# dmlc/difacto

Measured on AMD Instinct MI355X. Metric: examples/sec (FM SGD worker step, Criteo-shape, V_dim=64), higher is better.
Workload: dtype f32

## Files before the change

### difacto_amd/capi.py

```python
import ctypes as C
import os

import numpy as np

_HERE = os.path.dirname(os.path.abspath(__file__))
LIB_PATH = os.environ.get("DIFACTO_HIP_LIB") or os.path.join(_HERE, "libdifacto_hip.so")

FEA_COUNT, WEIGHT, GRADIENT = 1, 2, 3
INIT_REFRAND, INIT_HASH = 0, 1
U64MAX = 2 ** 64 - 1

SYMBOLS = [
    "dfh_last_error", "dfh_updater_param_default", "dfh_ctx_create", "dfh_ctx_destroy", "dfh_ctx_sync",
    "dfh_ctx_stream", "dfh_ctx_device", "dfh_reverse_bytes", "dfh_encode_fea_grp_id", "dfh_table_create",
    "dfh_table_destroy", "dfh_table_size", "dfh_table_param", "dfh_table_bytes", "dfh_pull", "dfh_push",
    "dfh_table_export", "dfh_table_import", "dfh_fm_predict", "dfh_fm_calcgrad", "dfh_loss_evaluate",
    "dfh_auc_times_n", "dfh_batch_create", "dfh_batch_destroy", "dfh_batch_load_host", "dfh_batch_load_device",
    "dfh_localize", "dfh_batch_load_localized_host", "dfh_batch_get_localized", "dfh_batch_shape", "dfh_sgd_step",
    "dfh_batch_progress", "dfh_batch_get_pred", "dfh_row_stride", "dfh_shard_pull", "dfh_shard_push_count",
    "dfh_shard_push_grad", "dfh_batch_forward", "dfh_batch_backward", "dfh_batch_device_keys", "dfh_malloc",
    "dfh_free", "dfh_memcpy_h2d", "dfh_memcpy_d2h", "dfh_ctx_set_timing", "dfh_ctx_get_timing", "dfh_kernel_name",
    "dfh_table_warm_start", "dfh_ctx_set_pipeline", "dfh_batch_lookup", "dfh_localize_lookup", "dfh_rowbuf_create", "dfh_rowbuf_destroy", "dfh_rowbuf_load_host", "dfh_batch_gather_rows", "dfh_batch_set_option", "dfh_batch_key_ranges", "dfh_batch_attach_device",
    "dfh_batch_key_ranges_device", "dfh_shard_resolve", "dfh_shard_pull_resolved", "dfh_shard_push_count_resolved",
    "dfh_shard_push_grad_resolved", "dfh_table_check", "dfh_ctx_set_timing_mask", "dfh_table_save", "dfh_table_load", "dfh_shard_resolve_multi", "dfh_shard_push_count_multi",
    "dfh_shard_push_grad_multi", "dfh_shard_count_pull_multi", "dfh_shard_push_grad_listed", "dfh_shard_release", "dfh_ctx_set_option", "dfh_table_set_has_aux", "dfh_table_has_aux",
    "dfh_comm_unique_id", "dfh_comm_create_rccl", "dfh_comm_create_callback", "dfh_comm_destroy", "dfh_comm_rank", "dfh_comm_world",
    "dfh_comm_allreduce_sum", "dfh_shard_create", "dfh_shard_destroy", "dfh_shard_owned_range", "dfh_shard_step", "dfh_shard_prefetch_counts",
    "dfh_shard_pull_host", "dfh_shard_push_host", "dfh_comm_allgather", "dfh_shard_balanced_splits", "dfh_shard_set_exchange", "dfh_shard_set_timing", "dfh_shard_get_timing",
    "dfh_comm_stats", "dfh_comm_info", "dfh_comm_selfcheck", "dfh_comm_wire_probe", "dfh_table_capacity", "dfh_batch_prepare_rows", "dfh_rowbuf_load_host_slices",
    "dfh_rowbuf_set_labels", "dfh_batch_prepare_cached", "dfh_batch_get_rows",
    "dfh_batch_create_many", "dfh_shard_multi_words", "dfh_shard_reserve", "dfh_comm_create_loopback", "dfh_comm_loopback_feed", "dfh_comm_loopback_wire", "dfh_comm_loopback_wire_time",
    "dfh_vec_inner_multi", "dfh_vec_combine", "dfh_vec_line_step", "dfh_lbfgs_create", "dfh_lbfgs_destroy", "dfh_lbfgs_add_chunk",
    "dfh_lbfgs_init_model", "dfh_lbfgs_shape", "dfh_lbfgs_get_model", "dfh_lbfgs_set_weights", "dfh_lbfgs_calc_grad",
# ... 625 lines not shown
    def load_localized_host(self, offset, index, value, label, feaids, feacnt=None):
        offset = np.ascontiguousarray(offset, np.uint64)
        index = np.ascontiguousarray(index, np.uint32)
        value = None if value is None else np.ascontiguousarray(value, np.float32)
        label = np.ascontiguousarray(label, np.float32)
        feaids = np.ascontiguousarray(feaids, np.uint64)
        feacnt = None if feacnt is None else np.ascontiguousarray(feacnt, np.float32)
        _ck(lib().dfh_batch_load_localized_host(self.h, len(offset) - 1, _p(offset), _p(index), _p(value), _p(label),
                                                _p(feaids), _p(feacnt), len(feaids)))

    def shape(self, want_U=True):
        a, b, c = C.c_size_t(0), C.c_size_t(0), C.c_size_t(0)
        _ck(lib().dfh_batch_shape(self.h, C.byref(a), C.byref(b), C.byref(c) if want_U else None))
        return a.value, b.value, c.value

    def get_localized(self):
        nrows, nnz, U = self.shape()
        feaids = np.zeros(max(U, 1), np.uint64)
        cnt = np.zeros(max(U, 1), np.float32)
        index = np.zeros(max(nnz, 1), np.uint32)
        u = C.c_size_t(0)
        _ck(lib().dfh_batch_get_localized(self.h, C.byref(u), _p(feaids), _p(cnt), _p(index)))
        return dict(U=U, feaids=feaids[:U], feacnt=cnt[:U], index=index[:nnz])

    def get_rows(self):
        nrows, _, _ = self.shape(want_U=False)
        off = np.zeros(nrows + 1, np.uint32)
        lab = np.zeros(nrows, np.float32)
        _ck(lib().dfh_batch_get_rows(self.h, _p(off), _p(lab)))
        return off, lab
# ... 428 lines not shown
```

### difacto_amd/csrc/dfh_api.hip

```cpp
#include <algorithm>
#include <chrono>
#include <cstring>
#include <mutex>
#include <new>
#include <thread>

#include <hip/hip_ext.h>
#include <rocprim/rocprim.hpp>

#include "dfh_kernels.hip"
#include "dfh_localize.hip"
#include "dfh_update.hip"
#include "dfh_riders.hip"

using namespace dfh;

namespace dfh {
static thread_local std::string g_err;
void set_error(const std::string& msg) { g_err = msg; }
}

struct dfh_ctx {
  int device = 0;
  hipStream_t stream = nullptr;
// ... 10 lines not shown
  int num_cu = 256;
  int fwd_depth = 5;
  int fwd_blocks = 0;
  int bwd_small_blocks = 2048;
  int upd_kernel = 1;
  int upd_hot_blocks = 512, upd_mid_blocks = 512, upd_few_blocks = 1024, upd_single_blocks = 4096;
  int upd_interleave = 0;
  int owner_per_key = 0;
  int upd_split = 1;
  int auc_in_update = 1;
  int shard_mixed_update = 1;
  int grow_initial_rows = 1 << 20;
  int event_flags = 1;
  int prep_priority = -1;
  int single_queue = 0;
  int rider_slot[4] = {2, 0, 1, 2};
  int rider_alone[4] = {0, 0, 0, 0};
  int rider_period[3] = {1, 1, 1};
  int rider_start[3] = {0, 0, 0};
  std::vector<dfh_batch*> pend;
  std::thread warm;

  uint32_t timing = 0;
  struct Span { int id; hipEvent_t a, b; int ride = 0; };
  std::vector<Span> spans;
  std::vector<hipEvent_t> pool;
  double t_ms[DFH_K_COUNT] = {0};
  uint64_t t_calls[DFH_K_COUNT] = {0};
};

// ... 111 lines not shown
  uint32_t auc_pending_n = 0;
  bool force_radix = false;
  bool force_sort_fallback = false;
  dfh_table* looked_up = nullptr;
  struct GatherSeg { struct dfh_rowbuf* rb; size_t at, n; };
  std::vector<GatherSeg> gsegs;
  GatherSrc gsrc{};
  bool gather_pending = false, gather_fusable = false, gather_any_value = false, loc_fuse_gather = false;
  const uint32_t *g_rows = nullptr, *g_off = nullptr;
  const float* g_lab = nullptr;
  LocView loc_v{};
  EmitOut loc_o{};
  uint32_t loc_gsort = 0;
  bool loc_big = false;
  int pend_stage = RID_STAGES;
};

namespace dfh {
namespace chunks {
inline hipError_t reset_prog(dfh_batch* b, hipStream_t s);
}
}

namespace {
int flush_pending(dfh_batch* b);
void pend_remove(dfh_ctx* c, dfh_batch* b);
inline hipStream_t prep_of(const dfh_batch* b) {
  const dfh_ctx* c = b->ctx;
  return (c->pipeline && b->prep) ? b->prep : c->stream;
}
// ... 820 lines not shown
  } else if (n == "shard_mixed_update") {
    DFH_ARG(value == 0 || value == 1, "shard_mixed_update must be 0 or 1");
    c->shard_mixed_update = value;
  } else if (n == "owner_per_key") {
    DFH_ARG(value == 0 || value == 1, "owner_per_key must be 0 (count push, Pull, gradient push per received entry) or 1 (per distinct key)");
    c->owner_per_key = value;
  } else if (n == "upd_split") {
    DFH_ARG(value == 0 || value == 1, "upd_split must be 0 (one block per hot key, whatever its length) or 1 (a block per part of 1 024 occurrences)");
    c->upd_split = value;
  } else if (n == "upd_interleave") {
    DFH_ARG(value >= 0 && value <= 64, "upd_interleave must be in [0, 64]");
    c->upd_interleave = value;
  } else if (n == "event_flags") {
    DFH_ARG(value == 0 || value == 1, "event_flags must be 0 (default events) or 1 (no system-scope fence); set before batches are created");
    c->event_flags = value;
  } else if (n == "single_queue") {
    DFH_ARG(value == 0 || value == 1, "single_queue must be 0 (preparation streams) or 1 (the Localizer's stages ride in the step's launches)");
    if (value != c->single_queue) {
      for (dfh_batch* p : std::vector<dfh_batch*>(c->pend)) {
        int rcf = flush_pending(p);
        if (rcf) return rcf;
      }
      int rcs = sync_all(c);
      if (rcs) return rcs;
      if (value) {
        c->nprep = 0;
        c->next_prep = 0;
        c->pipeline = false;
      }
      c->single_queue = value;
// ... 1138 lines not shown
}

int dfh_batch_destroy(dfh_batch* b) {
  if (b && b->n_prof)
    fprintf(stderr, "dfh_batch_prepare_rows x %llu: begin %.4f s, wait staged %.4f, write description %.4f, gather %.4f, localize %.4f, lookup + ready %.4f\n",
            (unsigned long long)b->n_prof, b->t_prof[0], b->t_prof[1], b->t_prof[2], b->t_prof[3], b->t_prof[4], b->t_prof[5]);
  if (!b) return DFH_OK;
  hipSetDevice(b->ctx->device);
  pend_remove(b->ctx, b);
  sync_all(b->ctx);
  if (b->ev_ready) hipEventDestroy(b->ev_ready);
  if (b->ev_free) hipEventDestroy(b->ev_free);
  if (b->ev_staged) hipEventDestroy(b->ev_staged);
  if (b->h_stage) hipHostFree(b->h_stage);
  if (b->d_xv) hipFree(b->d_xv);
  if (b->arena) hipFree(b->arena);
  if (b->shared_arena) {
    SharedArena* sa = static_cast<SharedArena*>(b->shared_arena);
    if (--sa->refs == 0) {
      hipFree(sa->base);
      delete sa;
    }
  }
  delete b;
  return DFH_OK;
}

}

#include "dfh_textparse.hip"
// ... 74 lines not shown
      else if (b->loc_fuse_gather) hipLaunchKernelGGL(k_loc_count_gather<LOC_MAX_BUCKETS>, dim3(v.ntiles), dim3(LOC_TILE_THREADS), 0, s, v, b->gsrc);
      else hipLaunchKernelGGL(k_loc_count<LOC_MAX_BUCKETS>, dim3(v.ntiles), dim3(LOC_TILE_THREADS), 0, s, v);
      break;
    case RID_SCATTER:
      if (b->loc_big) hipLaunchKernelGGL(k_loc_scatter<LOC_BIG_BUCKETS>, dim3(v.ntiles), dim3(LOC_TILE_THREADS), 0, s, v);
      else hipLaunchKernelGGL(k_loc_scatter<LOC_MAX_BUCKETS>, dim3(v.ntiles), dim3(LOC_TILE_THREADS), 0, s, v);
      break;
    case RID_SORT:
      hipLaunchKernelGGL(k_loc_sort, dim3(b->loc_gsort), dim3(LOC_SORT_THREADS), loc_sort_smem(), s, v);
      break;
    default:
      if (probe) hipLaunchKernelGGL(k_loc_emit<true>, dim3(b->loc_gsort), dim3(LOC_EMIT_THREADS), 0, s, v, b->loc_o, probe->v, b->d_urow);
      else hipLaunchKernelGGL(k_loc_emit<false>, dim3(b->loc_gsort), dim3(LOC_EMIT_THREADS), 0, s, v, b->loc_o, TableView{}, (uint32_t*)nullptr);
      break;
  }
}

void pend_remove(dfh_ctx* c, dfh_batch* b) {
  auto it = std::find(c->pend.begin(), c->pend.end(), b);
  if (it != c->pend.end()) c->pend.erase(it);
}

int flush_pending(dfh_batch* b) {
  dfh_ctx* c = b->ctx;
  if (b->pend_stage >= RID_STAGES) return DFH_OK;
  {
    TimeScope ts(c, DFH_K_LOCALIZE);
    for (int st = b->pend_stage; st < RID_STAGES; ++st) launch_loc_stage(b, st, c->stream);
  }
  b->pend_stage = RID_STAGES;
// ... 55 lines not shown
}

int localize_impl(dfh_batch* b, uint64_t max_index, dfh_table* probe) {
  dfh_ctx* c = b->ctx;
  DFH_HIP(hipSetDevice(c->device));
  const uint32_t N = (uint32_t)b->nnz;
  if (probe && N) {
    if (int rcr = table_reserve(probe, N)) return rcr;
  }
  {
    int rc = prep_begin(b);
    if (rc) return rc;
  }
  hipStream_t s = prep_of(b);
  b->looked_up = nullptr;
  if (b->pend_stage < RID_STAGES) {
    int rc = flush_pending(b);
    if (rc) return rc;
  }
  if (N == 0) {
    if (b->gather_pending) {
      int rcg = gather_alone(b, s);
      if (rcg) return rcg;
    }
    DFH_HIP(hipMemsetAsync(b->d_U, 0, 64 * sizeof(uint32_t), s));
    DFH_HIP(hipMemsetAsync(b->d_col_ptr, 0, 4, s));
    b->seg_nb = 0;
    b->localized = true;
    return prep_end(b);
  }
// ... 67 lines not shown
    o.sl.few = b->d_few;
    o.sl.few_ent = b->d_few_ent;
    v.split_n = b->d_U + 2;
    b->loc_big = big;
#ifndef DFH_LOC_GRID_CAP
#define DFH_LOC_GRID_CAP 1024
#endif
    b->loc_gsort = (unsigned)std::min<int>(P, big ? LOC_BIG_BUCKETS : DFH_LOC_GRID_CAP);
    if (cold && P > 1) {
      const uint32_t S = (uint32_t)P * LOC_OVERSAMPLE;
      const uint32_t nt = (S + 255) / 256;
      hipLaunchKernelGGL(k_ss_sample, dim3(nt), dim3(256), 0, s, v);
      hipLaunchKernelGGL(k_ss_rank, dim3(nt * nt), dim3(256), 0, s, v);
      hipLaunchKernelGGL(k_loc_splitters, dim3(nt), dim3(256), 0, s, v);
    }
    if (c->single_queue && !cold && !big && !probe) {
      b->pend_stage = 0;
      c->pend.push_back(b);
    } else {
      for (int st = 0; st < RID_STAGES; ++st) {
        launch_loc_stage(b, st, s, probe);
        if (st == RID_COUNT && b->loc_fuse_gather) {
          int rcg = gather_queued(b, s);
          b->loc_fuse_gather = false;
          if (rcg) return rcg;
        }
      }
    }
    b->spl_P = P;
    b->seg_nb = (uint32_t)P;
  } else {
// ... 153 lines not shown

int dfh_batch_shape(dfh_batch* b, size_t* nrows, size_t* nnz, size_t* U) {
  DFH_ARG(b, "NULL batch");
  if (nrows) *nrows = b->nrows;
  if (nnz) *nnz = b->nnz;
  if (U) {
    DFH_ARG(b->localized, "batch is not localized");
    uint32_t u = 0;
    int rc = flush_pending(b);
    if (rc) return rc;
    rc = sync_all(b->ctx);
    if (rc) return rc;
    DFH_HIP(hipMemcpyAsync(&u, b->d_U, 4, hipMemcpyDeviceToHost, b->ctx->stream));
    DFH_HIP(hipStreamSynchronize(b->ctx->stream));
    *U = u;
  }
  return DFH_OK;
}

int dfh_batch_get_localized(dfh_batch* b, size_t* U, uint64_t* feaids, float* feacnt, uint32_t* index) {
  DFH_ARG(b && b->localized, "batch is not localized");
  size_t u = 0;
  int rc = dfh_batch_shape(b, nullptr, nullptr, &u);
  if (rc) return rc;
  if (U) *U = u;
  hipStream_t s = b->ctx->stream;
  if (feaids && u) DFH_HIP(hipMemcpyAsync(feaids, b->d_feaids, u * 8, hipMemcpyDeviceToHost, s));
  if (feacnt && u) {
    if (!b->has_cnt) {
      hipLaunchKernelGGL(k_loc_counts, dim3(grid_for_threads(u, b->ctx)), dim3(256), 0, s, b->d_col_ptr, b->d_U, b->d_feacnt);
// ... 241 lines not shown
```

### difacto_amd/csrc/dfh_localize.hip

```cpp
#ifndef DFH_LOCALIZE_HIP_
#define DFH_LOCALIZE_HIP_
#include "dfh_internal.h"
#include "dfh_feed_layout.h"

namespace dfh {

constexpr int LOC_OVERSAMPLE = 8;
constexpr int LOC_MAX_BUCKETS = 1024;
constexpr int LOC_BIG_BUCKETS = 4096;
constexpr int LOC_AVG_BUCKET = 384;
constexpr int LOC_MIN_AVG = 48;
constexpr int LOC_MAX_AVG = 700;
constexpr int LOC_LDS_CAP = 1024;
#ifndef DFH_LOC_TILE_THREADS
#define DFH_LOC_TILE_THREADS 1024
#endif
constexpr int LOC_TILE_THREADS = DFH_LOC_TILE_THREADS;
constexpr int LOC_PER_THREAD = LOC_TILE / LOC_TILE_THREADS;
constexpr int LOC_SORT_THREADS = 256;
constexpr int LOC_EMIT_THREADS = 256;

struct LocView {
  const uint64_t* raw;
  uint32_t n;
// ... 23 lines not shown
  uint64_t* last_key;
  uint32_t* nheads;
  uint32_t* lh;
  uint32_t* split_n;
};

struct SegListsOut {
  uint2* mid;
  SegEnt* mid_ent;
  uint2* hot;
  SegEnt* hot_ent;
  uint2* few;
  SegEnt* few_ent;
};

__device__ __forceinline__ uint64_t make_key(uint64_t id, uint64_t max_index) {
  const uint64_t m = (max_index == ~0ULL) ? (id == ~0ULL ? 0ULL : id) : id % max_index;
  return reverse_bytes(m);
}

constexpr int LOC_XCDS = 8;

__device__ __forceinline__ bool comp_less(uint64_t ka, uint32_t pa, uint64_t kb, uint32_t pb) {
  return ka < kb || (ka == kb && pa < pb);
}

template <bool MAX>
__device__ __forceinline__ uint32_t wave_inclusive(uint32_t x) {
#define DFH_DPP_STEP(ctrl, row_mask)                                                                      \
  {                                                                                                       \
// ... 219 lines not shown
    v.run_off[bid * P + b] = h ? atomicAdd(&v.btotal[(bid & (LOC_XCDS - 1)) * MAXB + b], h) : 0u;
  }
}

template <int MAXB>
__global__ void __launch_bounds__(LOC_TILE_THREADS) k_loc_count(LocView v) {
  __shared__ __attribute__((aligned(16))) char smem[loc_count_smem<MAXB>()];
  loc_count_block<MAXB, LOC_TILE_THREADS>(v, blockIdx.x, gridDim.x, smem);
}
template <int MAXB>
__global__ void __launch_bounds__(LOC_TILE_THREADS) k_loc_count_gather(LocView v, GatherSrc g) {
  __shared__ __attribute__((aligned(16))) char smem[loc_count_smem<MAXB>() + loc_gather_smem()];
  loc_count_block<MAXB, LOC_TILE_THREADS, true>(v, blockIdx.x, gridDim.x, smem, &g);
}

__global__ void __launch_bounds__(LOC_DESC_ROWS) k_loc_describe(const uint32_t* __restrict__ src_off, const float* __restrict__ src_lab,
                                                                const uint32_t* __restrict__ h_rows, const uint32_t* __restrict__ h_base,
                                                                uint32_t n, uint32_t* __restrict__ dst_off, float* __restrict__ dst_lab,
                                                                int write_end) {
  __shared__ uint32_t wsum[LOC_DESC_ROWS / 64];
  const uint32_t q = blockIdx.x * LOC_DESC_ROWS + threadIdx.x;
  const bool in = q < n;
  const uint32_t r = h_rows[in ? q : n - 1u];
  const uint32_t lo = src_off[r], hi = src_off[r + 1u];
  const float lab = src_lab[r];
  const uint32_t len = in ? hi - lo : 0u;
  const uint32_t at = h_base[blockIdx.x] + block_exclusive_scan<LOC_DESC_ROWS / 64>(len, wsum, nullptr);
  if (in) {
    dst_off[q] = at;
    dst_lab[q] = lab;
// ... 118 lines not shown
    khi = take ? ohi : khi;
    tag = take ? ot : tag;
  }
}
template <int K, int J>
__device__ __forceinline__ void loc_net_merge(uint32_t& klo, uint32_t& khi, uint32_t& tag) {
  loc_net_stage<K, J>(klo, khi, tag);
  if constexpr (J > 1) loc_net_merge<K, J / 2>(klo, khi, tag);
}
template <int K = 2>
__device__ __forceinline__ void loc_net_sort64(uint32_t& klo, uint32_t& khi, uint32_t& tag) {
  loc_net_merge<K, K / 2>(klo, khi, tag);
  if constexpr (K < 64) loc_net_sort64<K * 2>(klo, khi, tag);
}

__device__ __forceinline__ bool loc_sort_bucket_lds(const LocView& v, uint32_t beg, uint32_t n, uint64_t* ak, uint32_t* ap,
                                                    uint64_t* bk, uint32_t* bp) {
  const uint64_t* gk = v.bkeys + beg;
  const uint32_t* gp = v.bpos + beg;
  uint64_t* sk = bk;
  uint32_t* sp = bp;
  const uint32_t lane = threadIdx.x & 63;
  for (uint32_t c0 = (threadIdx.x >> 6) * 64; c0 < n; c0 += LOC_SORT_THREADS) {
    const uint32_t idx = c0 + lane;
    const bool valid = idx < n;
    const uint64_t mk = valid ? gk[idx] : ~0ULL;
    uint32_t klo = (uint32_t)mk, khi = (uint32_t)(mk >> 32);
    uint32_t mp = valid ? gp[idx] : ~0u;
    loc_net_sort64(klo, khi, mp);
    if (valid) {
      bk[idx] = ((uint64_t)khi << 32) | klo;
      bp[idx] = mp;
    }
  }
  __syncthreads();
  constexpr int E = LOC_LDS_CAP / LOC_SORT_THREADS;
  constexpr int G = 2;
  static_assert(E * LOC_SORT_THREADS == LOC_LDS_CAP && E % G == 0 && LOC_SORT_THREADS % 64 == 0,
                "a thread carries E elements of a full bucket, G at a time");
  uint64_t* dk = ak;
  uint32_t* dp = ap;
  uint32_t sh = 6;
  for (uint32_t L = 64; L < n; L <<= 1, ++sh) {
// ... 27 lines not shown
      for (int e = 0; e < G; ++e) {
        const uint32_t idx = threadIdx.x + (g + e) * LOC_SORT_THREADS;
        if (idx < n) {
          const uint32_t dst = idx + at[e] - min((idx & ~(L - 1u)) | L, n);
          dk[dst] = mk[e];
          dp[dst] = mp[e];
        }
      }
    }
    __syncthreads();
    uint64_t* tk = sk; sk = dk; dk = tk;
    uint32_t* tp = sp; sp = dp; dp = tp;
  }
  return sk == ak;
}
__device__ __forceinline__ void loc_sort_bucket_global(const LocView& v, uint32_t beg, uint32_t n) {
  uint64_t* xk = v.bkeys + beg;
  uint32_t* xp = v.bpos + beg;
  uint64_t* yk = v.skeys + beg;
  uint32_t* yp = v.spos + beg;
  const uint32_t lane = threadIdx.x & 63;
  for (uint32_t c0 = (threadIdx.x >> 6) * 64; c0 < n; c0 += LOC_SORT_THREADS) {
    const uint32_t idx = c0 + lane;
    const bool valid = idx < n;
    const uint64_t mk = valid ? xk[idx] : ~0ULL;
    const uint32_t mp = valid ? xp[idx] : ~0u;
    const uint32_t lim = min(64u, n - c0);
    uint32_t rank = 0;
    for (uint32_t j = 0; j < lim; ++j) rank += comp_less(xk[c0 + j], xp[c0 + j], mk, mp) ? 1u : 0u;
    if (valid) {
      yk[c0 + rank] = mk;
      yp[c0 + rank] = mp;
    }
  }
  __syncthreads();
// ... 15 lines not shown
      const uint32_t dst = pair_base + (idx - r * L) + (lo - sib_beg);
      dstk[dst] = mk;
      dstp[dst] = mp;
    }
    __syncthreads();
    uint64_t* tk = srck; srck = dstk; dstk = tk;
    uint32_t* tp = srcp; srcp = dstp; dstp = tp;
  }
  if (srck != yk) {
    for (uint32_t t = threadIdx.x; t < n; t += blockDim.x) {
      yk[t] = srck[t];
      yp[t] = srcp[t];
    }
  }
  __syncthreads();
}

struct BucketSummary {
  uint32_t nheads, lh;
  uint64_t first_key, last_key;
};
template <bool WRITE>
__device__ __forceinline__ BucketSummary loc_bucket_summary(const uint64_t* sk, const uint32_t* sp, uint32_t n, uint64_t* ok,
                                                            uint32_t* op, uint32_t (*red)[LOC_SORT_THREADS / 64]) {
  uint32_t cnt = 0, last = 0;
  uint32_t t0 = threadIdx.x;
  asm volatile("" : "+v"(t0));
  for (uint32_t t = t0; t < n; t += LOC_SORT_THREADS) {
    const uint64_t k = sk[t];
    if (WRITE) {
// ... 16 lines not shown
  r.nheads = 1;
  r.lh = 0;
  r.first_key = 0;
  r.last_key = 0;
  if (threadIdx.x == 0) {
    for (int w = 0; w < LOC_SORT_THREADS / 64; ++w) {
      r.nheads += red[0][w];
      r.lh = max(r.lh, red[1][w]);
    }
    r.first_key = sk[0];
    r.last_key = sk[n - 1];
  }
  return r;
}

__device__ __forceinline__ void loc_sort_block(const LocView& v, const uint32_t bid, const uint32_t nblk, char* smem) {
  uint64_t* ak = reinterpret_cast<uint64_t*>(smem);
  uint64_t* bk = ak + LOC_LDS_CAP;
  uint32_t* ap = reinterpret_cast<uint32_t*>(bk + LOC_LDS_CAP);
  uint32_t* bp = ap + LOC_LDS_CAP;
  uint32_t (*red)[LOC_SORT_THREADS / 64] = reinterpret_cast<uint32_t (*)[LOC_SORT_THREADS / 64]>(bp + LOC_LDS_CAP);
  for (uint32_t b = bid; b < (uint32_t)v.P; b += nblk) {
    __syncthreads();
    const uint32_t beg = v.bstart[b], end = v.bstart[b + 1];
    const uint32_t n = end - beg;
    if (threadIdx.x < LOC_XCDS) v.btotal[threadIdx.x * v.bstride + b] = 0;
    if (n == 0) {
      if (threadIdx.x == 0) {
        v.nheads[b] = 0;
        v.lh[b] = 0;
        v.first_key[b] = 0;
        v.last_key[b] = 0;
      }
      continue;
    }
    BucketSummary sm;
    if (n <= LOC_LDS_CAP && !v.force_global) {
      const bool in_a = loc_sort_bucket_lds(v, beg, n, ak, ap, bk, bp);
      sm = loc_bucket_summary<true>(in_a ? ak : bk, in_a ? ap : bp, n, v.skeys + beg, v.spos + beg, red);
    } else {
      loc_sort_bucket_global(v, beg, n);
      sm = loc_bucket_summary<false>(v.skeys + beg, v.spos + beg, n, nullptr, nullptr, red);
    }
    if (threadIdx.x == 0) {
      v.nheads[b] = sm.nheads;
      v.lh[b] = sm.lh;
      v.first_key[b] = sm.first_key;
      v.last_key[b] = sm.last_key;
    }
  }
}
__global__ void __launch_bounds__(LOC_SORT_THREADS) k_loc_sort(LocView v) {
  extern __shared__ __attribute__((aligned(16))) char smem[];
  loc_sort_block(v, blockIdx.x, gridDim.x, smem);
}

template <int NW, bool PROBE>
__device__ __forceinline__ void loc_emit_bucket(const LocView& v, uint32_t b, uint32_t beg, uint32_t n, const uint64_t* sk,
                                                const uint32_t* sp, uint32_t cont, uint32_t ubase, uint32_t carry1,
                                                const float* __restrict__ value,
                                                uint64_t* __restrict__ feaids, uint32_t* __restrict__ col_ptr,
                                                uint32_t* __restrict__ index, uint32_t* __restrict__ s_row,
                                                float* __restrict__ s_val, uint32_t* __restrict__ d_U, const SegListsOut& sl,
                                                uint32_t* wsum, uint32_t* wmax, uint32_t* n_mid, uint32_t* n_hot,
                                                uint32_t* n_few, const TableView& tab, uint32_t* __restrict__ urow) {
  const uint32_t P = (uint32_t)v.P;
  const uint32_t moff = beg / (BWD_SMALL + 1) + 2 * b, hoff = beg / (BWD_MID + 1) + 2 * b, foff = beg / 2 + 2 * b;
  uint32_t run_heads = 0, run_max1 = carry1;
  for (uint32_t base = 0; base < n; base += blockDim.x) {
// ... 132 lines not shown
    uint32_t ubase, carry_all;
    block_exclusive_scan<NW>(part, wsum, &ubase);
    block_exclusive_max<NW>(carry1, wmax, &carry_all);
    __syncthreads();
    loc_emit_bucket<NW, PROBE>(v, b, beg, n, v.skeys + beg, v.spos + beg, sh_cont, ubase, carry_all, o.value, o.feaids, o.col_ptr,
                               o.index, o.s_row, o.s_val, o.d_U, sl, wsum, wmax, &n_mid, &n_hot, &n_few, tab, urow);
  }
}

template <bool PROBE>
__global__ void __launch_bounds__(LOC_EMIT_THREADS) k_loc_emit(LocView v, EmitOut o, TableView tab, uint32_t* __restrict__ urow) {
  __shared__ __attribute__((aligned(16))) char smem[loc_emit_smem()];
  loc_emit_block<PROBE>(v, o, tab, urow, blockIdx.x, gridDim.x, smem);
}

}
#endif
```

### include/difacto_hip.h

```cpp
#ifndef DIFACTO_HIP_H_
#define DIFACTO_HIP_H_
#include <stddef.h>
#include <stdint.h>

#ifdef __cplusplus
extern "C" {
#endif

enum {
  DFH_OK = 0,
  DFH_ERR_ARG = 1,
  DFH_ERR_HIP = 2,
  DFH_ERR_CAPACITY = 3,
  DFH_ERR_STATE = 4
};

enum { DFH_FEA_COUNT = 1, DFH_WEIGHT = 2, DFH_GRADIENT = 3 };

enum {
  DFH_INIT_REFRAND = 0,
  DFH_INIT_HASH = 1
};

typedef struct {
// ... 109 lines not shown
} dfh_slice;
int dfh_rowbuf_load_slices(dfh_rowbuf* rb, size_t nrows, const size_t* offset, int nslices, const dfh_slice* slices);
int dfh_batch_gather_rows(dfh_batch* b, size_t nrows, const size_t* offset, const float* label, int nseg, dfh_rowbuf* const* bufs,
                          const uint32_t* const* rows, const size_t* seg_rows);
int dfh_batch_prepare_rows(dfh_table* t, dfh_batch* b, size_t nrows, const size_t* offset, const float* label, int nseg,
                           dfh_rowbuf* const* bufs, const uint32_t* const* rows, const size_t* seg_rows, uint64_t max_index);
int dfh_rowbuf_set_labels(dfh_rowbuf* rb, size_t nrows, const float* label);
int dfh_batch_prepare_cached(dfh_table* t, dfh_batch* b, size_t nrows, int nseg, dfh_rowbuf* const* bufs, const uint32_t* const* rows,
                             const size_t* seg_rows, uint64_t max_index);

int dfh_batch_load_localized_host(dfh_batch* b, size_t nrows, const size_t* offset, const uint32_t* index,
                                  const float* value, const float* label, const uint64_t* feaids,
                                  const float* feacnt, size_t U);
int dfh_batch_get_localized(dfh_batch* b, size_t* U, uint64_t* feaids, float* feacnt, uint32_t* index);
int dfh_batch_shape(dfh_batch* b, size_t* nrows, size_t* nnz, size_t* U);
int dfh_batch_get_rows(dfh_batch* b, uint32_t* offset, float* label);

int dfh_sgd_step(dfh_table* t, dfh_batch* b, int is_train, int push_cnt);
int dfh_batch_progress(dfh_batch* b, dfh_progress* out, int reset);
int dfh_batch_get_pred(dfh_batch* b, float* pred);
int dfh_batch_split_entries(dfh_batch* b, uint32_t* n);

size_t dfh_row_stride(int V_dim);
int dfh_shard_pull(dfh_table* t, const uint64_t* d_keys, size_t n, float* d_rows);
int dfh_shard_push_count(dfh_table* t, const uint64_t* d_keys, size_t n, const float* d_cnt);
int dfh_shard_push_grad(dfh_table* t, const uint64_t* d_keys, size_t n, const float* d_grads);
int dfh_batch_forward(dfh_batch* b, int V_dim, const float* d_rows);
int dfh_batch_backward(dfh_batch* b, int V_dim, const float* d_rows, float* d_grads);
int dfh_batch_device_keys(dfh_batch* b, const uint64_t** d_feaids, const float** d_feacnt, size_t* U);
int dfh_batch_key_ranges(dfh_batch* b, int nparts, uint32_t* bounds);
// ... 111 lines not shown
```

Baseline: 88.76 million.

## Place keys directly into per-bucket slabs, replacing count/scatter passes in Localizer

Adds a placed form of the Localizer that runs on warm calls of the small size class: a single kernel computes keys, row tags and bucket ids, then writes each key straight into a fixed per-bucket, per-XCD sub-slab, with overflow going to a side list. This replaces the separate count and scatter passes. The sort and emit kernels are given placed variants that read these slabs through a slot map, and buckets that overflow are compacted into a spill region. It is on by default (loc_place=1) and is meant to save one full pass over the keys plus a kernel launch, at the cost of extra device memory and a slower path for skewed buckets that overflow.

```diff
diff --git a/difacto_amd/capi.py b/difacto_amd/capi.py
--- a/difacto_amd/capi.py
+++ b/difacto_amd/capi.py
@@ -16,7 +16,7 @@
     "dfh_table_destroy", "dfh_table_size", "dfh_table_param", "dfh_table_bytes", "dfh_pull", "dfh_push",
     "dfh_table_export", "dfh_table_import", "dfh_fm_predict", "dfh_fm_calcgrad", "dfh_loss_evaluate",
     "dfh_auc_times_n", "dfh_batch_create", "dfh_batch_destroy", "dfh_batch_load_host", "dfh_batch_load_device",
-    "dfh_localize", "dfh_batch_load_localized_host", "dfh_batch_get_localized", "dfh_batch_shape", "dfh_sgd_step",
+    "dfh_localize", "dfh_batch_load_localized_host", "dfh_batch_get_localized", "dfh_batch_shape", "dfh_batch_loc_stats", "dfh_sgd_step",
     "dfh_batch_progress", "dfh_batch_get_pred", "dfh_row_stride", "dfh_shard_pull", "dfh_shard_push_count",
     "dfh_shard_push_grad", "dfh_batch_forward", "dfh_batch_backward", "dfh_batch_device_keys", "dfh_malloc",
     "dfh_free", "dfh_memcpy_h2d", "dfh_memcpy_d2h", "dfh_ctx_set_timing", "dfh_ctx_get_timing", "dfh_kernel_name",
@@ -672,6 +672,13 @@
         _ck(lib().dfh_batch_shape(self.h, C.byref(a), C.byref(b), C.byref(c) if want_U else None))
         return a.value, b.value, c.value
 
+    def loc_stats(self):
+        fn = lib().dfh_batch_loc_stats
+        fn.argtypes = [C.c_void_p, C.POINTER(C.c_uint32)]
+        out = (C.c_uint32 * 4)()
+        _ck(fn(self.h, out))
+        return tuple(int(x) for x in out)
+
     def get_localized(self):
         nrows, nnz, U = self.shape()
         feaids = np.zeros(max(U, 1), np.uint64)
diff --git a/difacto_amd/csrc/dfh_api.hip b/difacto_amd/csrc/dfh_api.hip
--- a/difacto_amd/csrc/dfh_api.hip
+++ b/difacto_amd/csrc/dfh_api.hip
@@ -48,6 +48,7 @@
   int event_flags = 1;
   int prep_priority = -1;
   int single_queue = 0;
+  int loc_place = 1;
   int rider_slot[4] = {2, 0, 1, 2};
   int rider_alone[4] = {0, 0, 0, 0};
   int rider_period[3] = {1, 1, 1};
@@ -189,6 +190,9 @@
   uint32_t loc_gsort = 0;
   bool loc_big = false;
   int pend_stage = RID_STAGES;
+  void* place_mem = nullptr;
+  PlaceView loc_p{};
+  int loc_form = 0;
 };
 
 namespace dfh {
@@ -1039,6 +1043,9 @@
   } else if (n == "event_flags") {
     DFH_ARG(value == 0 || value == 1, "event_flags must be 0 (default events) or 1 (no system-scope fence); set before batches are created");
     c->event_flags = value;
+  } else if (n == "loc_place") {
+    DFH_ARG(value == 0 || value == 1, "loc_place must be 0 (count, scatter, sort, emit) or 1 (place, sort, emit on a warm call of the small size class)");
+    c->loc_place = value;
   } else if (n == "single_queue") {
     DFH_ARG(value == 0 || value == 1, "single_queue must be 0 (preparation streams) or 1 (the Localizer's stages ride in the step's launches)");
     if (value != c->single_queue) {
@@ -2207,6 +2214,7 @@
   if (b->ev_staged) hipEventDestroy(b->ev_staged);
   if (b->h_stage) hipHostFree(b->h_stage);
   if (b->d_xv) hipFree(b->d_xv);
+  if (b->place_mem) hipFree(b->place_mem);
   if (b->arena) hipFree(b->arena);
   if (b->shared_arena) {
     SharedArena* sa = static_cast<SharedArena*>(b->shared_arena);
@@ -2311,6 +2319,39 @@
       else hipLaunchKernelGGL(k_loc_emit<false>, dim3(b->loc_gsort), dim3(LOC_EMIT_THREADS), 0, s, v, b->loc_o, TableView{}, (uint32_t*)nullptr);
       break;
   }
+}
+
+int ensure_place(dfh_batch* b, hipStream_t s) {
+  if (b->place_mem) return DFH_OK;
+  const size_t slab = (size_t)LOC_MAX_BUCKETS * LOC_LDS_CAP, N = b->max_nnz, E = slab + N;
+  auto al = [](size_t bytes) { return (bytes + 255) & ~(size_t)255; };
+  const size_t need = 2 * al(E * 8) + 2 * al(E * 4) + al(N * 8) + 2 * al(N * 4) + al((size_t)LOC_MAX_BUCKETS * 8) + 2 * 256;
+  DFH_ARG(E < 0xFFFFFFF0ULL, "batch too large for the Localizer's placed form");
+  DFH_HIP(hipMalloc(&b->place_mem, need));
+  char* at = static_cast<char*>(b->place_mem);
+  auto take = [&](size_t bytes) { char* r = at; at += al(bytes); return r; };
+  PlaceView& p = b->loc_p;
+  p.pkeys = reinterpret_cast<uint64_t*>(take(E * 8));
+  p.skeys = reinterpret_cast<uint64_t*>(take(E * 8));
+  p.ptags = reinterpret_cast<uint32_t*>(take(E * 4));
+  p.stags = reinterpret_cast<uint32_t*>(take(E * 4));
+  p.spill0 = (uint32_t)slab;
+  p.ovf_key = reinterpret_cast<uint64_t*>(take(N * 8));
+  p.ovf_tag = reinterpret_cast<uint32_t*>(take(N * 4));
+  p.ovf_b = reinterpret_cast<uint32_t*>(take(N * 4));
+  p.bdesc = reinterpret_cast<uint2*>(take((size_t)LOC_MAX_BUCKETS * 8));
+  p.cnt = reinterpret_cast<uint32_t*>(take(256));
+  p.stats = reinterpret_cast<uint32_t*>(take(256));
+  DFH_HIP(hipMemsetAsync(p.cnt, 0, 512, s));
+  return DFH_OK;
+}
+
+void launch_loc_placed(dfh_batch* b, hipStream_t s) {
+  const LocView& v = b->loc_v;
+  hipLaunchKernelGGL(k_loc_place<LOC_MAX_BUCKETS>, dim3(v.ntiles), dim3(LOC_TILE_THREADS), 0, s, v, b->loc_p);
+  hipLaunchKernelGGL(k_loc_sort_placed, dim3(b->loc_gsort), dim3(LOC_SORT_THREADS), loc_sort_smem(), s, v, b->loc_p);
+  hipLaunchKernelGGL(k_loc_emit_placed<false>, dim3(b->loc_gsort), dim3(LOC_EMIT_THREADS), 0, s, v, b->loc_p, b->loc_o, TableView{},
+                     (uint32_t*)nullptr);
 }
 
 void pend_remove(dfh_ctx* c, dfh_batch* b) {
@@ -2396,6 +2437,7 @@
   }
   hipStream_t s = prep_of(b);
   b->looked_up = nullptr;
+  b->loc_form = 0;
   if (b->pend_stage < RID_STAGES) {
     int rc = flush_pending(b);
     if (rc) return rc;
@@ -2493,7 +2535,14 @@
       hipLaunchKernelGGL(k_ss_rank, dim3(nt * nt), dim3(256), 0, s, v);
       hipLaunchKernelGGL(k_loc_splitters, dim3(nt), dim3(256), 0, s, v);
     }
-    if (c->single_queue && !cold && !big && !probe) {
+    const bool placed = c->loc_place && !cold && !big && !c->single_queue && !probe && !b->loc_fuse_gather &&
+                        v.ntiles >= 2 * LOC_XCDS;
+    if (placed) {
+      int rcp = ensure_place(b, s);
+      if (rcp) return rcp;
+      launch_loc_placed(b, s);
+      b->loc_form = 1;
+    } else if (c->single_queue && !cold && !big && !probe) {
       b->pend_stage = 0;
       c->pend.push_back(b);
     } else {
@@ -2677,6 +2726,24 @@
     DFH_HIP(hipMemcpyAsync(&u, b->d_U, 4, hipMemcpyDeviceToHost, b->ctx->stream));
     DFH_HIP(hipStreamSynchronize(b->ctx->stream));
     *U = u;
+  }
+  return DFH_OK;
+}
+
+int dfh_batch_loc_stats(dfh_batch* b, uint32_t out[4]) {
+  DFH_ARG(b && out, "dfh_batch_loc_stats: NULL argument");
+  DFH_ARG(b->localized, "batch is not localized");
+  out[0] = (uint32_t)b->loc_form;
+  out[1] = out[2] = out[3] = 0;
+  if (b->loc_form == 1) {
+    int rc = sync_all(b->ctx);
+    if (rc) return rc;
+    uint32_t st[3] = {0, 0, 0};
+    DFH_HIP(hipMemcpyAsync(st, b->loc_p.stats, sizeof(st), hipMemcpyDeviceToHost, b->ctx->stream));
+    DFH_HIP(hipStreamSynchronize(b->ctx->stream));
+    out[1] = st[2];
+    out[2] = st[0];
+    out[3] = st[1];
   }
   return DFH_OK;
 }
diff --git a/difacto_amd/csrc/dfh_localize.hip b/difacto_amd/csrc/dfh_localize.hip
--- a/difacto_amd/csrc/dfh_localize.hip
+++ b/difacto_amd/csrc/dfh_localize.hip
@@ -61,6 +61,22 @@
   SegEnt* few_ent;
 };
 
+constexpr int LOC_CX = 128;
+constexpr int LOC_PLACE_ROWS = 256;
+struct PlaceView {
+  uint64_t* pkeys;
+  uint32_t* ptags;
+  uint64_t* skeys;
+  uint32_t* stags;
+  uint32_t spill0;
+  uint64_t* ovf_key;
+  uint32_t* ovf_tag;
+  uint32_t* ovf_b;
+  uint32_t* cnt;
+  uint32_t* stats;
+  uint2* bdesc;
+};
+
 __device__ __forceinline__ uint64_t make_key(uint64_t id, uint64_t max_index) {
   const uint64_t m = (max_index == ~0ULL) ? (id == ~0ULL ? 0ULL : id) : id % max_index;
   return reverse_bytes(m);
@@ -310,6 +326,127 @@
   loc_count_block<MAXB, LOC_TILE_THREADS, true>(v, blockIdx.x, gridDim.x, smem, &g);
 }
 
+template <int MAXB>
+constexpr size_t loc_place_smem() { return loc_count_smem<MAXB>() + (size_t)(LOC_PLACE_ROWS + 1) * 4 + 4; }
+
+template <int MAXB, int THREADS>
+__device__ __forceinline__ void loc_place_block(const LocView& v, const PlaceView& p, const uint32_t bid, char* smem) {
+  constexpr int PER = LOC_TILE / THREADS;
+  static_assert(PER * THREADS == LOC_TILE, "a tile is a whole number of elements per thread");
+  static_assert(LOC_CX * LOC_XCDS == LOC_LDS_CAP, "a bucket's slab is one sub-slab per XCD group");
+  uint64_t* sk = reinterpret_cast<uint64_t*>(smem);
+  uint32_t* sp = reinterpret_cast<uint32_t*>(smem + (size_t)MAXB * 8);
+  uint32_t* hist = sp + MAXB;
+  uint32_t* roff = hist + MAXB;
+  uint32_t* sh_r0 = roff + LOC_PLACE_ROWS + 1;
+  const int P = v.P;
+  const uint32_t base = bid * LOC_TILE;
+  if (threadIdx.x < 64) {
+    uint32_t lo = 0, hi = v.nrows;
+    while (hi - lo > 1u) {
+      const uint32_t step = ((hi - lo - 1u) >> 6) + 1u;
+      const uint64_t q = (uint64_t)lo + (uint64_t)(threadIdx.x + 1u) * step;
+      const bool ok = q < hi && v.offset[q] <= base;
+      const uint32_t c = (uint32_t)__popcll(__ballot(ok));
+      hi = min(hi, lo + (c + 1u) * step);
+      lo += c * step;
+    }
+    if (threadIdx.x == 0) *sh_r0 = lo;
+  }
+  for (int b = threadIdx.x; b < P; b += THREADS) {
+    hist[b] = 0;
+    sk[b] = b < P - 1 ? v.spl_key[b] : ~0ULL;
+    sp[b] = b < P - 1 ? v.spl_pos[b] : ~0u;
+  }
+  if (bid == 0 && threadIdx.x == 0 && v.split_n) *v.split_n = 0u;
+  __syncthreads();
+  const uint32_t r0 = *sh_r0;
+  const uint32_t nst = min((uint32_t)LOC_PLACE_ROWS, v.nrows - r0);
+  for (uint32_t q = threadIdx.x; q <= nst; q += THREADS) roff[q] = v.offset[r0 + q];
+  uint64_t key[PER];
+#pragma unroll
+  for (int e = 0; e < PER; ++e) {
+    const uint32_t i = base + e * THREADS + threadIdx.x;
+    key[e] = i < v.n ? make_key(v.raw[i], v.max_index) : ~0ULL;
+  }
+  __syncthreads();
+  uint32_t tag[PER];
+#pragma unroll
+  for (int e = 0; e < PER; ++e) {
+    const uint32_t i = base + e * THREADS + threadIdx.x;
+    tag[e] = 0;
+    if (i < v.n) {
+      uint32_t lo, hi;
+      if (i < roff[nst]) {
+        lo = 0;
+        hi = nst - 1u;
+        while (lo < hi) {
+          const uint32_t mid = (lo + hi + 1u) >> 1;
+          if (roff[mid] <= i) lo = mid; else hi = mid - 1u;
+        }
+        lo += r0;
+      } else {
+        lo = r0 + nst;
+        hi = v.nrows - 1u;
+        while (lo < hi) {
+          const uint32_t mid = lo + ((hi - lo + 1u) >> 1);
+          if (v.offset[mid] <= i) lo = mid; else hi = mid - 1u;
+        }
+      }
+      tag[e] = (i << v.tb) | (lo & ((1u << v.tb) - 1u));
+    }
+  }
+  int lo[PER], hi[PER];
+#pragma unroll
+  for (int e = 0; e < PER; ++e) { lo[e] = 0; hi[e] = P - 1; }
+  for (int step = P; step > 1; step = (step + 1) >> 1) {
+#pragma unroll
+    for (int e = 0; e < PER; ++e) {
+      if (lo[e] < hi[e]) {
+        const uint32_t i = base + e * THREADS + threadIdx.x;
+        const int mid = (lo[e] + hi[e]) >> 1;
+        if (comp_less(key[e], i << v.tb, sk[mid], sp[mid])) hi[e] = mid; else lo[e] = mid + 1;
+      }
+    }
+  }
+  uint32_t rk[PER];
+#pragma unroll
+  for (int e = 0; e < PER; ++e) {
+    const uint32_t i = base + e * THREADS + threadIdx.x;
+    rk[e] = i < v.n ? atomicAdd(&hist[lo[e]], 1u) : 0u;
+  }
+  __syncthreads();
+  const uint32_t xcd = bid & (LOC_XCDS - 1);
+  for (int b = threadIdx.x; b < P; b += THREADS) {
+    const uint32_t h = hist[b];
+    if (h) hist[b] = atomicAdd(&v.btotal[xcd * MAXB + b], h);
+  }
+  __syncthreads();
+#pragma unroll
+  for (int e = 0; e < PER; ++e) {
+    const uint32_t i = base + e * THREADS + threadIdx.x;
+    if (i < v.n) {
+      const uint32_t slot = hist[lo[e]] + rk[e];
+      if (slot < (uint32_t)LOC_CX) {
+        const uint32_t at = ((uint32_t)lo[e] * LOC_XCDS + xcd) * LOC_CX + slot;
+        p.pkeys[at] = key[e];
+        p.ptags[at] = tag[e];
+      } else {
+        const uint32_t j = atomicAdd(&p.cnt[0], 1u);
+        p.ovf_key[j] = key[e];
+        p.ovf_tag[j] = tag[e];
+        p.ovf_b[j] = (uint32_t)lo[e];
+      }
+    }
+  }
+}
+
+template <int MAXB>
+__global__ void __launch_bounds__(LOC_TILE_THREADS) k_loc_place(LocView v, PlaceView p) {
+  __shared__ __attribute__((aligned(16))) char smem[loc_place_smem<MAXB>()];
+  loc_place_block<MAXB, LOC_TILE_THREADS>(v, p, blockIdx.x, smem);
+}
+
 __global__ void __launch_bounds__(LOC_DESC_ROWS) k_loc_describe(const uint32_t* __restrict__ src_off, const float* __restrict__ src_lab,
                                                                 const uint32_t* __restrict__ h_rows, const uint32_t* __restrict__ h_base,
                                                                 uint32_t n, uint32_t* __restrict__ dst_off, float* __restrict__ dst_lab,
@@ -458,19 +595,30 @@
   if constexpr (K < 64) loc_net_sort64<K * 2>(klo, khi, tag);
 }
 
-__device__ __forceinline__ bool loc_sort_bucket_lds(const LocView& v, uint32_t beg, uint32_t n, uint64_t* ak, uint32_t* ap,
-                                                    uint64_t* bk, uint32_t* bp) {
-  const uint64_t* gk = v.bkeys + beg;
-  const uint32_t* gp = v.bpos + beg;
+struct PlacedMap {
+  uint32_t pre[LOC_XCDS - 1];
+  uint32_t gap[LOC_XCDS - 1];
+  __device__ __forceinline__ uint32_t slot(uint32_t idx) const {
+    uint32_t s = idx;
+#pragma unroll
+    for (int x = 0; x < LOC_XCDS - 1; ++x) s += idx >= pre[x] ? gap[x] : 0u;
+    return s;
+  }
+};
+template <bool PLACED = false>
+__device__ __forceinline__ bool loc_sort_bucket_lds(const uint64_t* gk, const uint32_t* gp, uint32_t n, uint64_t* ak, uint32_t* ap,
+                                                    uint64_t* bk, uint32_t* bp, const PlacedMap* pm = nullptr) {
   uint64_t* sk = bk;
   uint32_t* sp = bp;
   const uint32_t lane = threadIdx.x & 63;
   for (uint32_t c0 = (threadIdx.x >> 6) * 64; c0 < n; c0 += LOC_SORT_THREADS) {
     const uint32_t idx = c0 + lane;
     const bool valid = idx < n;
-    const uint64_t mk = valid ? gk[idx] : ~0ULL;
+    uint32_t src = idx;
+    if constexpr (PLACED) src = pm->slot(idx);
+    const uint64_t mk = valid ? gk[src] : ~0ULL;
     uint32_t klo = (uint32_t)mk, khi = (uint32_t)(mk >> 32);
-    uint32_t mp = valid ? gp[idx] : ~0u;
+    uint32_t mp = valid ? gp[src] : ~0u;
     loc_net_sort64(klo, khi, mp);
     if (valid) {
       bk[idx] = ((uint64_t)khi << 32) | klo;
@@ -528,11 +676,7 @@
   }
   return sk == ak;
 }
-__device__ __forceinline__ void loc_sort_bucket_global(const LocView& v, uint32_t beg, uint32_t n) {
-  uint64_t* xk = v.bkeys + beg;
-  uint32_t* xp = v.bpos + beg;
-  uint64_t* yk = v.skeys + beg;
-  uint32_t* yp = v.spos + beg;
+__device__ __forceinline__ void loc_sort_bucket_global_at(uint64_t* xk, uint32_t* xp, uint64_t* yk, uint32_t* yp, uint32_t n) {
   const uint32_t lane = threadIdx.x & 63;
   for (uint32_t c0 = (threadIdx.x >> 6) * 64; c0 < n; c0 += LOC_SORT_THREADS) {
     const uint32_t idx = c0 + lane;
@@ -578,6 +722,10 @@
     }
   }
   __syncthreads();
+}
+
+__device__ __forceinline__ void loc_sort_bucket_global(const LocView& v, uint32_t beg, uint32_t n) {
+  loc_sort_bucket_global_at(v.bkeys + beg, v.bpos + beg, v.skeys + beg, v.spos + beg, n);
 }
 
 struct BucketSummary {
@@ -624,7 +772,9 @@
   return r;
 }
 
-__device__ __forceinline__ void loc_sort_block(const LocView& v, const uint32_t bid, const uint32_t nblk, char* smem) {
+template <bool PLACED = false>
+__device__ __forceinline__ void loc_sort_block(const LocView& v, const uint32_t bid, const uint32_t nblk, char* smem,
+                                               const PlaceView* pp = nullptr) {
   uint64_t* ak = reinterpret_cast<uint64_t*>(smem);
   uint64_t* bk = ak + LOC_LDS_CAP;
   uint32_t* ap = reinterpret_cast<uint32_t*>(bk + LOC_LDS_CAP);
@@ -632,37 +782,110 @@
   uint32_t (*red)[LOC_SORT_THREADS / 64] = reinterpret_cast<uint32_t (*)[LOC_SORT_THREADS / 64]>(bp + LOC_LDS_CAP);
   for (uint32_t b = bid; b < (uint32_t)v.P; b += nblk) {
     __syncthreads();
-    const uint32_t beg = v.bstart[b], end = v.bstart[b + 1];
-    const uint32_t n = end - beg;
-    if (threadIdx.x < LOC_XCDS) v.btotal[threadIdx.x * v.bstride + b] = 0;
-    if (n == 0) {
+    if constexpr (!PLACED) {
+      const uint32_t beg = v.bstart[b], end = v.bstart[b + 1];
+      const uint32_t n = end - beg;
+      if (threadIdx.x < LOC_XCDS) v.btotal[threadIdx.x * v.bstride + b] = 0;
+      if (n == 0) {
+        if (threadIdx.x == 0) {
+          v.nheads[b] = 0;
+          v.lh[b] = 0;
+          v.first_key[b] = 0;
+          v.last_key[b] = 0;
+        }
+        continue;
+      }
+      BucketSummary sm;
+      if (n <= LOC_LDS_CAP && !v.force_global) {
+        const bool in_a = loc_sort_bucket_lds(v.bkeys + beg, v.bpos + beg, n, ak, ap, bk, bp);
+        sm = loc_bucket_summary<true>(in_a ? ak : bk, in_a ? ap : bp, n, v.skeys + beg, v.spos + beg, red);
+      } else {
+        loc_sort_bucket_global(v, beg, n);
+        sm = loc_bucket_summary<false>(v.skeys + beg, v.spos + beg, n, nullptr, nullptr, red);
+      }
       if (threadIdx.x == 0) {
-        v.nheads[b] = 0;
-        v.lh[b] = 0;
-        v.first_key[b] = 0;
-        v.last_key[b] = 0;
-      }
-      continue;
-    }
-    BucketSummary sm;
-    if (n <= LOC_LDS_CAP && !v.force_global) {
-      const bool in_a = loc_sort_bucket_lds(v, beg, n, ak, ap, bk, bp);
-      sm = loc_bucket_summary<true>(in_a ? ak : bk, in_a ? ap : bp, n, v.skeys + beg, v.spos + beg, red);
+        v.nheads[b] = sm.nheads;
+        v.lh[b] = sm.lh;
+        v.first_key[b] = sm.first_key;
+        v.last_key[b] = sm.last_key;
+      }
     } else {
-      loc_sort_bucket_global(v, beg, n);
-      sm = loc_bucket_summary<false>(v.skeys + beg, v.spos + beg, n, nullptr, nullptr, red);
-    }
-    if (threadIdx.x == 0) {
-      v.nheads[b] = sm.nheads;
-      v.lh[b] = sm.lh;
-      v.first_key[b] = sm.first_key;
-      v.last_key[b] = sm.last_key;
+      const PlaceView& p = *pp;
+      PlacedMap pm;
+      uint32_t n = 0, over = 0;
+#pragma unroll
+      for (int x = 0; x < LOC_XCDS; ++x) {
+        const uint32_t t = (uint32_t)__builtin_amdgcn_readfirstlane((int)v.btotal[x * v.bstride + b]);
+        const uint32_t c = min(t, (uint32_t)LOC_CX);
+        over += t - c;
+        n += c;
+        if (x < LOC_XCDS - 1) {
+          pm.pre[x] = n;
+          pm.gap[x] = (uint32_t)LOC_CX - c;
+        }
+      }
+      const uint32_t ntot = n + over;
+      if (ntot == 0) {
+        if (threadIdx.x == 0) {
+          v.nheads[b] = 0;
+          v.lh[b] = 0;
+          v.first_key[b] = 0;
+          v.last_key[b] = 0;
+          p.bdesc[b] = make_uint2(0u, 0u);
+        }
+        continue;
+      }
+      const uint32_t slab = b * (uint32_t)LOC_LDS_CAP;
+      uint32_t where = slab;
+      BucketSummary sm;
+      if (over == 0 && ntot <= LOC_LDS_CAP && !v.force_global) {
+        const bool in_a = loc_sort_bucket_lds<true>(p.pkeys + slab, p.ptags + slab, ntot, ak, ap, bk, bp, &pm);
+        sm = loc_bucket_summary<true>(in_a ? ak : bk, in_a ? ap : bp, ntot, p.skeys + slab, p.stags + slab, red);
+      } else {
+        if (threadIdx.x == 0) {
+          red[0][0] = atomicAdd(&p.cnt[1], ntot);
+          red[1][0] = 0;
+          atomicAdd(&p.cnt[2], 1u);
+        }
+        __syncthreads();
+        where = p.spill0 + (uint32_t)__builtin_amdgcn_readfirstlane((int)red[0][0]);
+        for (uint32_t t = threadIdx.x; t < n; t += LOC_SORT_THREADS) {
+          const uint32_t src = slab + pm.slot(t);
+          p.pkeys[where + t] = p.pkeys[src];
+          p.ptags[where + t] = p.ptags[src];
+        }
+        if (over) {
+          const uint32_t listed = p.cnt[0];
+          for (uint32_t j = threadIdx.x; j < listed; j += LOC_SORT_THREADS) {
+            if (p.ovf_b[j] == b) {
+              const uint32_t at = where + n + atomicAdd(&red[1][0], 1u);
+              p.pkeys[at] = p.ovf_key[j];
+              p.ptags[at] = p.ovf_tag[j];
+            }
+          }
+        }
+        __syncthreads();
+        loc_sort_bucket_global_at(p.pkeys + where, p.ptags + where, p.skeys + where, p.stags + where, ntot);
+        sm = loc_bucket_summary<false>(p.skeys + where, p.stags + where, ntot, nullptr, nullptr, red);
+      }
+      if (threadIdx.x < LOC_XCDS) v.btotal[threadIdx.x * v.bstride + b] = 0;
+      if (threadIdx.x == 0) {
+        v.nheads[b] = sm.nheads;
+        v.lh[b] = sm.lh;
+        v.first_key[b] = sm.first_key;
+        v.last_key[b] = sm.last_key;
+        p.bdesc[b] = make_uint2(ntot, where);
+      }
     }
   }
 }
 __global__ void __launch_bounds__(LOC_SORT_THREADS) k_loc_sort(LocView v) {
   extern __shared__ __attribute__((aligned(16))) char smem[];
   loc_sort_block(v, blockIdx.x, gridDim.x, smem);
+}
+__global__ void __launch_bounds__(LOC_SORT_THREADS) k_loc_sort_placed(LocView v, PlaceView p) {
+  extern __shared__ __attribute__((aligned(16))) char smem[];
+  loc_sort_block<true>(v, blockIdx.x, gridDim.x, smem, &p);
 }
 
 template <int NW, bool PROBE>
@@ -825,5 +1048,79 @@
   loc_emit_block<PROBE>(v, o, tab, urow, blockIdx.x, gridDim.x, smem);
 }
 
+template <bool PROBE>
+__device__ __forceinline__ void loc_emit_placed_block(const LocView& v, const PlaceView& p, const EmitOut& o, const TableView& tab,
+                                                      uint32_t* __restrict__ urow, const uint32_t bid, const uint32_t nblk, char* smem) {
+  constexpr int NW = LOC_EMIT_THREADS / 64;
+  constexpr int BPT = LOC_MAX_BUCKETS / LOC_EMIT_THREADS;
+  static_assert(BPT * LOC_EMIT_THREADS == LOC_MAX_BUCKETS, "every thread owns the same number of buckets");
+  uint32_t* wsum = reinterpret_cast<uint32_t*>(smem);
+  uint32_t* wmax = wsum + NW;
+  uint32_t& sh_cont = wmax[NW];
+  uint32_t& n_mid = wmax[NW + 1];
+  uint32_t& n_hot = wmax[NW + 2];
+  uint32_t& n_few = wmax[NW + 3];
+  const SegListsOut& sl = o.sl;
+  const uint32_t P = (uint32_t)v.P;
+  if (bid == 0 && threadIdx.x < 3) {
+    p.stats[threadIdx.x] = p.cnt[threadIdx.x];
+    p.cnt[threadIdx.x] = 0;
+  }
+  for (uint32_t b = bid; b < P; b += nblk) {
+    __syncthreads();
+    const uint2 own = p.bdesc[b];
+    const uint32_t n = own.x;
+    if (threadIdx.x == 0) {
+      n_mid = 0;
+      n_hot = 0;
+      n_few = 0;
+      if (n == 0) {
+        sl.mid[b] = make_uint2(0u, 0u);
+        sl.hot[b] = make_uint2(0u, 0u);
+        sl.few[b] = make_uint2(0u, 0u);
+      }
+    }
+    if (n == 0) continue;
+    uint32_t q0 = threadIdx.x * BPT;
+    asm volatile("" : "+v"(q0));
+    uint32_t sum = 0;
+#pragma unroll
+    for (int j = 0; j < BPT; ++j) sum += q0 + j < b ? p.bdesc[q0 + j].x : 0u;
+    uint32_t beg;
+    uint32_t bq = block_exclusive_scan<NW>(sum, wsum, &beg);
+    uint32_t part = 0, carry1 = 0;
+#pragma unroll 1
+    for (uint32_t q = q0; q < q0 + BPT && q <= b; ++q) {
+      const uint32_t nn = q < b ? p.bdesc[q].x : n;
+      if (nn == 0) continue;
+      int pr = (int)q - 1;
+      while (pr >= 0 && p.bdesc[pr].x == 0) --pr;
+      const uint32_t c = (pr >= 0 && v.first_key[q] == v.last_key[pr]) ? 1u : 0u;
+      if (q == b) {
+        sh_cont = c;
+      } else {
+        part += v.nheads[q] - c;
+        const uint32_t l = v.lh[q];
+        if (l > 0) carry1 = max(carry1, bq + l + 1);
+        else if (!c) carry1 = max(carry1, bq + 1);
+        bq += nn;
+      }
+    }
+    uint32_t ubase, carry_all;
+    block_exclusive_scan<NW>(part, wsum, &ubase);
+    block_exclusive_max<NW>(carry1, wmax, &carry_all);
+    __syncthreads();
+    loc_emit_bucket<NW, PROBE>(v, b, beg, n, p.skeys + own.y, p.stags + own.y, sh_cont, ubase, carry_all, o.value, o.feaids,
+                               o.col_ptr, o.index, o.s_row, o.s_val, o.d_U, sl, wsum, wmax, &n_mid, &n_hot, &n_few, tab, urow);
+  }
+}
+
+template <bool PROBE>
+__global__ void __launch_bounds__(LOC_EMIT_THREADS) k_loc_emit_placed(LocView v, PlaceView p, EmitOut o, TableView tab,
+                                                                      uint32_t* __restrict__ urow) {
+  __shared__ __attribute__((aligned(16))) char smem[loc_emit_smem()];
+  loc_emit_placed_block<PROBE>(v, p, o, tab, urow, blockIdx.x, gridDim.x, smem);
+}
+
 }
 #endif
diff --git a/include/difacto_hip.h b/include/difacto_hip.h
--- a/include/difacto_hip.h
+++ b/include/difacto_hip.h
@@ -147,6 +147,7 @@
                                   const float* feacnt, size_t U);
 int dfh_batch_get_localized(dfh_batch* b, size_t* U, uint64_t* feaids, float* feacnt, uint32_t* index);
 int dfh_batch_shape(dfh_batch* b, size_t* nrows, size_t* nnz, size_t* U);
+int dfh_batch_loc_stats(dfh_batch* b, uint32_t out[4]);
 int dfh_batch_get_rows(dfh_batch* b, uint32_t* offset, float* label);
 
 int dfh_sgd_step(dfh_table* t, dfh_batch* b, int is_train, int push_cnt);
```

Result: slower. 87.75 million (-1.1%).
